# sherna90/dropout_hamiltonian_montecarlo

Hardware: AMD Instinct MI355X
Metric: leapfrog-steps/sec × param-dim, MNIST softmax SGHMC, 1/2/4/8 chains↔GPUs (higher is better)
Workload: dtype f64

## Files before the change

### dropout_hamiltonian_montecarlo_amd/_native.py

```python
import atexit
import ctypes
import os
import threading

import torch

_HERE = os.path.dirname(os.path.abspath(__file__))
LIB_PATH = os.path.join(_HERE, "lib", os.environ.get("HMCX_LIB", "libhmcx.so"))

HMCX_F32, HMCX_F64 = 0, 1
NOISE_BUFFER, NOISE_PHILOX = 0, 1

c_int, c_double, c_void_p = ctypes.c_int, ctypes.c_double, ctypes.c_void_p
c_i64p = ctypes.POINTER(ctypes.c_int64)
c_i32p = ctypes.POINTER(ctypes.c_int32)
c_dblp = ctypes.POINTER(ctypes.c_double)
c_u8p = ctypes.POINTER(ctypes.c_uint8)


class SamplerArgs(ctypes.Structure):
    _fields_ = [("dtype", c_int), ("B", c_int), ("D", c_int), ("K", c_int), ("C", c_int),
                ("n_steps", c_int), ("alpha", c_double), ("log_prior", c_double),
                ("X", c_void_p), ("Y", c_void_p), ("row0", c_void_p), ("eps", c_void_p),
                ("n_iter", c_void_p), ("u_accept", c_void_p), ("want_ll", c_void_p),
# ... 92 lines not shown
    _fields_ = [("dim", c_int), ("C", c_int), ("n_steps", c_int), ("mu", c_void_p), ("prec", c_void_p),
                ("nlp_const", c_double), ("mult", c_dblp), ("site", c_i32p), ("u_accept", c_dblp),
                ("noise_mode", c_int), ("noise", c_void_p), ("noise_off", c_i64p),
                ("seed", ctypes.c_uint64), ("chain0", ctypes.c_uint32), ("step_base", ctypes.c_uint32),
                ("x", c_void_p), ("out_A", c_void_p), ("out_accepted", c_void_p), ("out_logp", c_void_p),
                ("out_E", c_void_p), ("out_trace", c_void_p)]


MODEL_SOFTMAX, MODEL_LOGISTIC = 0, 1
MLP_MASK_SLOT0 = 0x80000000
MLP_MASKS_NONE, MLP_MASKS_FIXED, MLP_MASKS_PHILOX = 0, 1, 2


EXPORTS = ("hmcx_version", "hmcx_create", "hmcx_destroy", "hmcx_last_error", "hmcx_set_stream",
           "hmcx_synchronize", "hmcx_set_graph_mode", "hmcx_set_sghmc_path", "hmcx_set_timing", "hmcx_get_timing",
           "hmcx_philox_uniforms", "hmcx_philox_normals", "hmcx_philox_normals_f64",
           "hmcx_softmax_grad", "hmcx_softmax_loglik", "hmcx_softmax_predict", "hmcx_sghmc_run",
           "hmcx_sgld_run", "hmcx_hmc_mvn_run", "hmcx_mlp_masks", "hmcx_mlp_grad", "hmcx_mlp_loss",
           "hmcx_mlp_sghmc_run", "hmcx_mlp_hmc_leapfrog", "hmcx_mlp_predictive", "hmcx_logistic_grad", "hmcx_logistic_loglik", "hmcx_logistic_predict",
           "hmcx_sumsq", "hmcx_sgd_run", "hmcx_hmc_run", "hmcx_hmc_chains_run", "hmcx_mh_run", "hmcx_mh_mvn_run", "hmcx_axpy", "hmcx_mvn_eval",
           "hmcx_clear_abort", "hmcx_get_recoveries", "hmcx_note_recovery", "hmcx_get_mlp_forward_counts", "hmcx_set_sgld_fuse", "hmcx_philox_schedule", "hmcx_host_wait", "hmcx_set_mlp_fuse",
           "hmcx_comm_unique_id", "hmcx_comm_init", "hmcx_comm_destroy", "hmcx_allgather_chain_stats",
           "hmcx_allreduce_f64", "hmcx_chain_diagnostics", "hmcx_p2_plan_query", "hmcx_p2_ahead_query",
           "hmcx_set_sghmc_ahead", "hmcx_sghmc_ahead_note", "hmcx_p2_ahead_rule", "hmcx_sghmc_batch_plan_query")

_lib = None
_lock = threading.Lock()


class HmcxError(RuntimeError):
    pass


def load_library():
    global _lib
    with _lock:
        if _lib is not None:
            return _lib
        if not os.path.exists(LIB_PATH):
            raise HmcxError("libhmcx.so not built (%s): run `python -c 'import __graft_entry__ as g; g.build()'`"
                            % LIB_PATH)
        lib = ctypes.CDLL(LIB_PATH)
        lib.hmcx_version.restype = c_int
        lib.hmcx_create.argtypes = [c_int, ctypes.POINTER(c_void_p)]
        lib.hmcx_destroy.argtypes = [c_void_p]
        lib.hmcx_last_error.argtypes = [c_void_p]
        lib.hmcx_last_error.restype = ctypes.c_char_p
# ... 57 lines not shown
        lib.hmcx_logistic_grad.argtypes = [c_void_p, c_int, c_void_p, c_void_p, c_int, c_int, c_int,
                                           c_void_p, c_void_p, c_double, c_void_p, c_void_p]
        lib.hmcx_logistic_loglik.argtypes = [c_void_p, c_int, c_void_p, c_void_p, c_int, c_int, c_int,
                                             c_void_p, c_void_p, c_void_p]
        lib.hmcx_logistic_predict.argtypes = [c_void_p, c_int, c_void_p, c_int, c_int, c_int, c_void_p, c_void_p,
                                              c_void_p]
        lib.hmcx_sumsq.argtypes = [c_void_p, c_int, c_void_p, ctypes.c_int64, c_void_p]
        lib.hmcx_sgd_run.argtypes = [c_void_p, ctypes.POINTER(SgdArgs)]
        lib.hmcx_hmc_run.argtypes = [c_void_p, ctypes.POINTER(HmcArgs)]
        if hasattr(lib, "hmcx_hmc_chains_run"):
            lib.hmcx_hmc_chains_run.argtypes = [c_void_p, ctypes.POINTER(HmcChainsArgs)]
        if hasattr(lib, "hmcx_mh_run"):
            lib.hmcx_mh_run.argtypes = [c_void_p, ctypes.POINTER(MhArgs)]
            lib.hmcx_mh_mvn_run.argtypes = [c_void_p, ctypes.POINTER(MhMvnArgs)]
        if hasattr(lib, "hmcx_p2_plan_query"):
            lib.hmcx_p2_plan_query.argtypes = [c_int, c_int, c_int, c_int, c_int, ctypes.c_longlong, c_int, c_int,
                                               ctypes.POINTER(ctypes.c_longlong)]
        if hasattr(lib, "hmcx_set_sghmc_ahead"):
            lib.hmcx_set_sghmc_ahead.argtypes = [c_void_p, c_int]
            lib.hmcx_sghmc_ahead_note.argtypes = [c_void_p, c_i32p, c_int]
            lib.hmcx_p2_ahead_rule.argtypes = [c_int, c_int, c_int]
            lib.hmcx_p2_ahead_query.argtypes = [c_int, c_int, c_int, c_int, c_int, ctypes.c_longlong, c_int, c_int,
                                                ctypes.POINTER(ctypes.c_longlong)]
        if hasattr(lib, "hmcx_sghmc_batch_plan_query"):
            lib.hmcx_sghmc_batch_plan_query.argtypes = [c_int] * 11 + [ctypes.POINTER(ctypes.c_longlong)]
        lib.hmcx_axpy.argtypes = [c_void_p, c_int, c_int, ctypes.c_int64, c_double, c_void_p, c_void_p]
        lib.hmcx_mvn_eval.argtypes = [c_void_p, c_int, c_int, c_void_p, c_void_p, c_double, c_void_p, c_void_p,
                                      c_void_p]
        _lib = lib
        return lib


class Context:

    def __init__(self, device):
        lib = load_library()
        if not torch.cuda.is_available():
            raise HmcxError("no HIP device visible: the HIP engine has no CPU fallback")
        self.lib = lib
        self.device = torch.device("cuda", device if isinstance(device, int) else (device.index or 0))
        h = c_void_p()
        with torch.cuda.device(self.device):
            rc = lib.hmcx_create(self.device.index, ctypes.byref(h))
        if rc != 0:
            raise HmcxError("hmcx_create failed (%d)" % rc)
        self.h = h
# ... 11 lines not shown

    def check(self, rc, what):
        if rc != 0:
            msg = self.lib.hmcx_last_error(self.h)
            raise HmcxError("%s failed (%d): %s" % (what, rc, msg.decode() if msg else ""))

    path = 0

    def set_sghmc_path(self, path):
        self.check(self.lib.hmcx_set_sghmc_path(self.h, int(path)), "hmcx_set_sghmc_path")
        self.path = int(path)

    def set_sghmc_ahead(self, mode):
        self.check(self.lib.hmcx_set_sghmc_ahead(self.h, int(mode)), "hmcx_set_sghmc_ahead")

    def sghmc_ahead_note(self, accepted):
        if not hasattr(self.lib, "hmcx_sghmc_ahead_note"):
            return
        if hasattr(accepted, "ctypes") and accepted.dtype.str == "<i4" and accepted.flags.c_contiguous:
            self.lib.hmcx_sghmc_ahead_note(self.h, accepted.ctypes.data_as(c_i32p), int(accepted.size))
            return
        flags = [1 if v else 0 for v in accepted]
        self.lib.hmcx_sghmc_ahead_note(self.h, (ctypes.c_int32 * len(flags))(*flags), len(flags))

    def clear_abort(self):
        self.check(self.lib.hmcx_clear_abort(self.h), "hmcx_clear_abort")

    RECOVERY_KINDS = ("persistent_sghmc", "mlp_fused", "sgld_wide_fused")

    def recoveries(self):
        if not hasattr(self.lib, "hmcx_get_recoveries"):
            return None
        out = (ctypes.c_int64 * len(self.RECOVERY_KINDS))()
        self.check(self.lib.hmcx_get_recoveries(self.h, out), "hmcx_get_recoveries")
        return dict(zip(self.RECOVERY_KINDS, (int(v) for v in out)))

    def note_recovery(self, kind):
        self.check(self.lib.hmcx_note_recovery(self.h, self.RECOVERY_KINDS.index(kind)), "hmcx_note_recovery")

    MLP_FORWARD_KINDS = ("fwdr", "batched", "single")

    def mlp_forward_counts(self):
        out = (ctypes.c_int64 * len(self.MLP_FORWARD_KINDS))()
        self.check(self.lib.hmcx_get_mlp_forward_counts(self.h, out), "hmcx_get_mlp_forward_counts")
        return dict(zip(self.MLP_FORWARD_KINDS, (int(v) for v in out)))

# ... 155 lines not shown
```

### dropout_hamiltonian_montecarlo_amd/csrc/hmcx_ctx.hip

```cpp
#include "hmcx_common.h"
#include "hmcx_internal.h"
#include <new>
#include <cstdio>
#include <cstring>
#include <cmath>

namespace hmcx {

int set_error(hmcx_ctx* ctx, int code, const std::string& msg) {
  if (ctx) ctx->err = msg;
  return code;
}

bool Workspace::retry() {
  if (off <= ctx->ws_cap) return false;
  if (ctx->ws) {
    if (hipDeviceSynchronize() != hipSuccess) { failed = true; return false; }
    (void)hipFree(ctx->ws);
    ctx->ws = nullptr;
    ctx->ws_cap = 0;
  }
  const size_t want = off + off / 4 + (1 << 20);
  if (hipMalloc((void**)&ctx->ws, want) != hipSuccess) {
    ctx->ws = nullptr;
// ... 528 lines not shown
  return HMCX_OK;
}

int hmcx_destroy(hmcx_ctx* ctx) {
  HMCX_GUARD_CTX(ctx);
  (void)hipSetDevice(ctx->device);
  (void)hipStreamSynchronize(ctx->stream);
  if (ctx->ws) (void)hipFree(ctx->ws);
  for (int i = 0; i < 2; ++i) {
    if (ctx->stage_buf[i]) (void)hipHostFree(ctx->stage_buf[i]);
    if (ctx->stage_evv[i]) (void)hipEventDestroy(ctx->stage_evv[i]);
  }
  if (ctx->ev_in) (void)hipEventDestroy(ctx->ev_in);
  for (auto& pr : ctx->t_pend) { (void)hipEventDestroy(pr.first); (void)hipEventDestroy(pr.second); }
  if (ctx->t_open) (void)hipEventDestroy(ctx->t_open);
  for (auto& pr : ctx->abort_pend) (void)hipEventDestroy(pr.first);
  for (auto e : ctx->ev_pool) (void)hipEventDestroy(e);
  for (auto& m : ctx->host_marks) (void)hipEventDestroy(m.second);
  for (auto e : ctx->host_mark_pool) (void)hipEventDestroy(e);
  if (ctx->abort_host) (void)hipHostFree(ctx->abort_host);
  if (ctx->abort_dev) (void)hipFree(ctx->abort_dev);
  if (ctx->mlp_abort_dev) (void)hipFree(ctx->mlp_abort_dev);
  if (ctx->wide_abort_dev) (void)hipFree(ctx->wide_abort_dev);
  if (ctx->zeros_dev) (void)hipFree(ctx->zeros_dev);
  if (ctx->gx_arena) (void)hipFree(ctx->gx_arena);
  if (ctx->pred_ws) (void)hipFree(ctx->pred_ws);
  for (auto& g : ctx->graveyard) {
    (void)hipGraphExecDestroy(g.first);
    (void)hipEventDestroy(g.second);
  }
  if (ctx->own_stream) (void)hipStreamDestroy(ctx->own_stream);
  delete ctx;
  return HMCX_OK;
}

const char* hmcx_last_error(const hmcx_ctx* ctx) { return ctx ? ctx->err.c_str() : "null context"; }

int hmcx_set_stream(hmcx_ctx* ctx, void* stream) {
  HMCX_GUARD_CTX(ctx);
  ctx->stream = (hipStream_t)stream;
  return HMCX_OK;
}

int hmcx_synchronize(hmcx_ctx* ctx) {
  HMCX_GUARD_CTX(ctx);
  HMCX_HIP(ctx, hipStreamSynchronize(ctx->stream));
// ... 545 lines not shown
```

### dropout_hamiltonian_montecarlo_amd/csrc/hmcx_internal.h

```cpp
#pragma once
#include <hip/hip_runtime.h>
#include <stdint.h>
#include <string>
#include <vector>
#include <algorithm>
#include "hmcx.h"

struct hmcx_ctx {
  int device = 0;
  hipStream_t own_stream = nullptr;
  hipStream_t stream = nullptr;
  std::string err;
  int graph_mode = 0;
  int sghmc_path = 0;
  int sghmc_ahead = 2;
  int ahead_on = 1;
  uint64_t ahead_flags = 0;
  int ahead_seen = 0;
  int num_cus = 256;
  size_t lds_max = 160 * 1024;
  char* ws = nullptr;
  size_t ws_cap = 0;
  char* stage_buf[2] = {nullptr, nullptr};
  size_t stage_capv[2] = {0, 0};
  hipEvent_t stage_evv[2] = {nullptr, nullptr};
  bool stage_pend[2] = {false, false};
  int stage_cur = 0;
  size_t stage_off = 0;
  char* gx_arena = nullptr;
  size_t gx_bytes = 0;
  unsigned gx_epoch = 0;
  std::vector<int64_t> rs_poff, rs_nzo;
  std::vector<double> sched_L, sched_u;
  std::vector<int32_t> sched_n;
  std::vector<std::pair<std::pair<const void*, int>, int>> occ_cache;
  hipEvent_t ev_in = nullptr, ev_out = nullptr;
  std::vector<std::pair<hipGraphExec_t, hipEvent_t>> graveyard;
  int timing = 0;
  hipEvent_t t_open = nullptr;
  std::vector<std::pair<hipEvent_t, hipEvent_t>> t_pend;
  double t_ms = 0.0;
// ... 179 lines not shown
```

### dropout_hamiltonian_montecarlo_amd/csrc/hmcx_p2x.h

```cpp
#pragma once
#include "hmcx_common.h"

namespace hmcx {

constexpr int QTH = 256;
constexpr int QNW = QTH / 64;
constexpr int QNPM = 16;
#ifndef HMCX_P2_SLEEP
#define HMCX_P2_SLEEP 1
#endif
constexpr unsigned long long QTIMEOUT = 400000000ull;

typedef unsigned int gran_t __attribute__((ext_vector_type(4)));
__host__ __device__ inline int p2_pad(int n, int pad) { return pad ? (n + 7) & ~7 : n; }

__device__ inline uint64_t opaque_s64(uint64_t x) {
  uint32_t lo = (uint32_t)x, hi = (uint32_t)(x >> 32);
  asm volatile("" : "+s"(lo), "+s"(hi));
  return ((uint64_t)hi << 32) | lo;
}
__device__ inline int opaque(int x) {
  asm volatile("" : "+v"(x));
  return x;
}
// ... 235 lines not shown
}
__device__ inline int p2_wait_decision(unsigned long long* w, unsigned ep, int* abort_flag) {
  unsigned long long t0 = __builtin_amdgcn_s_memrealtime();
  for (int spins = 0;; ++spins) {
    const unsigned long long cur = __hip_atomic_load(w, __ATOMIC_RELAXED, __HIP_MEMORY_SCOPE_AGENT);
    if ((cur >> 2) == (unsigned long long)ep) return (int)(cur & 3ull);
    if ((spins & 63) == 63 &&
        (__builtin_amdgcn_s_memrealtime() - t0 > QTIMEOUT ||
         __hip_atomic_load(abort_flag, __ATOMIC_RELAXED, __HIP_MEMORY_SCOPE_AGENT))) {
      const int d = p2_decide(w, ep, P2_ABORT);
      if (d == P2_ABORT) p2_timeout(abort_flag, -1, ep);
      return d;
    }
    if (HMCX_P2_SLEEP) __builtin_amdgcn_s_sleep(1);
  }
}

__device__ inline bool all_ok(bool ok, int* sh_fail) {
  if (!ok) *sh_fail = 1;
  __syncthreads();
  return *sh_fail == 0;
}

__device__ inline double wsum(double v, double* sh) {
#pragma unroll
  for (int m = 32; m >= 1; m >>= 1) v += __shfl_xor(v, m, 64);
  if ((threadIdx.x & 63) == 0) sh[threadIdx.x >> 6] = v;
  __syncthreads();
  double r = sh[0];
#pragma unroll
  for (int w = 1; w < QNW; ++w) r += sh[w];
  __syncthreads();
  return r;
}

template <int CTRL> __device__ inline double dpp64(double v) {
  const unsigned long long x = __builtin_bit_cast(unsigned long long, v);
  const int lo = __builtin_amdgcn_mov_dpp((int)(unsigned)x, CTRL, 0xF, 0xF, false);
  const int hi = __builtin_amdgcn_mov_dpp((int)(unsigned)(x >> 32), CTRL, 0xF, 0xF, false);
  return __builtin_bit_cast(double, (unsigned long long)(unsigned)lo | ((unsigned long long)(unsigned)hi << 32));
}
template <int CTRL> __device__ inline float dpp64(float v) {
  return __builtin_bit_cast(float, __builtin_amdgcn_mov_dpp(__builtin_bit_cast(int, v), CTRL, 0xF, 0xF, false));
}
constexpr int DPP_XOR1 = 0xB1, DPP_XOR2 = 0x4E, DPP_HMIRROR = 0x141, DPP_MIRROR = 0x140;
template <typename T> __device__ inline T g16_max2(T v) {
// ... 18 lines not shown
```

### dropout_hamiltonian_montecarlo_amd/csrc/hmcx_persist2.hip

```cpp
#include "hmcx_common.h"
#include "hmcx_internal.h"
#include "hmcx_persist.h"
#include "hmcx_p2x.h"
#include <cstdio>
#include <cstdlib>
#include <vector>

namespace hmcx {


struct Q2Args {
  int B, D, K, P, n_steps;
  int Gr, Gf, Br, Bf, BfP, BFP, Ro, Fo;
  double alpha, neg_inv_n, log_prior;
  const void* X; const void* Y;
  const double* eps; const double* u; const int64_t* row0; const int32_t* n_iter;
  int noise_mode; const double* noise; const int64_t* noff;
  uint64_t seed; uint32_t chain0, step_base;
  void* W; void* b;
  char* arena;
  int oXA, oXD, oXB, oXW, oXS;
  int oXC;
  int oXAh, oXQ, oXP;
  int help;
// ... 1 lines not shown
  int pad;
  unsigned ep0;
  int zoff;
  int spread;
  int xmap;
  int fl2;
  int al2;
  int prefetch;
  int acc1;
  int bar;
  int* abort_flag;
  int force_abort;
  double* out_A; int32_t* out_acc; double* out_ll; double* out_E;
  void* out_trace;
  void* out_mom;
  unsigned long long* prof;
  unsigned long long* trace;
  int* verdict;
  int ninl;
  struct { double eps, u; int64_t row0; int32_t n_iter, pad_; } inl[32];
  int ahead;
  int laneoff;
  int oXV;
};
constexpr int P2_NINL = 32;
__device__ inline int sched_k(int s) { return s < P2_NINL ? s : P2_NINL - 1; }
template <typename V>
__device__ inline V sched_at(bool inl, int s, V kv, const V* g) {
  const V gv = g[inl ? 0 : s];
  return inl ? kv : gv;
}

struct P2Verdict {
  int* out;
  bool done;
  __device__ ~P2Verdict() {
    if (out && !done) out[0] = 1;
  }
};
constexpr int P2TR_IT = 16;
#ifndef HMCX_P2_HELP_DEFAULT
#define HMCX_P2_HELP_DEFAULT 2
#endif

struct P2Prof {
  unsigned long long* out;
// ... 395 lines not shown
      }
    }
    verdict.done = true;
    return;
  }

  const int s_first = lanei, s_inc = ah ? 2 : 1;
  bool redo = false;
  bool pf_done = false;
  int tb = 0;
  const int perV = p2_pad(Fo * KC + KC, pad);
  const auto gatherQ = [&](int k) -> bool {
    const int ni = Fo * KC + KC;
    const int base0 = a.oXQ + ((k & 1) * Gf + f) * Gr * perV;
    const bool ok = gather_ws(rs, base0, perV, Gr, ni, [](int i) { return i; },
                              [&](int p, int i) { return i < Fo * KC ? p * Fo + i / KC < nfeat : p == 0; },
                              a.ep0 + (unsigned)k, a.abort_flag, [&](int q, double v) {
      const int p = q / ni, i = q - p * ni;
      if (i < Fo * KC) Wf[(p * Fo + i / KC) * 16 + i % KC] = (T)v;
      else bsh[i - Fo * KC] = (T)v;
    });
    return all_ok(ok, ish);
  };
  const auto waitV = [&](int k) -> int {
    if (threadIdx.x == 0) {
      const int g = (a.oXV + ((k & 1) * G + pbid) * 8) * 16;
      const unsigned tg = a.ep0 + (unsigned)k;
      unsigned long long t0 = __builtin_amdgcn_s_memrealtime();
      int res = -1;
      for (int spins = 0;; ++spins) {
        const gran_t v = __builtin_amdgcn_raw_buffer_load_b128(rs, g, 0, 16 );
        if (pass_complete(gran_miss(v, tg))) { res = decode(v) != 0.0 ? 1 : 0; break; }
        if ((spins & 63) == 63 && p2_spin_over(t0, a.abort_flag, a.oXV, tg)) break;
        __builtin_amdgcn_s_sleep(4);
      }
      ish[2] = res;
    }
    __syncthreads();
    const int res = ish[2];
    __syncthreads();
    return res;
  };

  for (int s = s_first; s < a.n_steps;) {
    const int tid = opaque((int)threadIdx.x), lane = tid & 63, wave = tid >> 6, lr = lane & 15;
    const double epsd = sched_at(inl, s, a.inl[sched_k(s)].eps, a.eps);
    const T eps = (T)epsd, ome = (T)(1.0 - epsd), nsc = (T)(2.0 * epsd);
    const int n = sched_at(inl, s, a.inl[sched_k(s)].n_iter, a.n_iter);
    const int64_t rw = sched_at(inl, s, a.inl[sched_k(s)].row0, a.row0);
    const T* Xg = reinterpret_cast<const T*>(a.X) + (size_t)rw * D;
    const T* Yg = reinterpret_cast<const T*>(a.Y) + (size_t)rw * K;
    prof.stamp(0);
    if (s == a.force_abort && bid == G - 1) {
      if (tid == 0) __hip_atomic_store(a.abort_flag, 1, __ATOMIC_RELAXED, __HIP_MEMORY_SCOPE_AGENT);
      return;
    }

    if ((s == s_first || !prefetch) && !redo) load_step_rows<T>(Xc, Yc, Xg, Yg, Br, BfP, BFP, nrow, nfeat, row0, feat0, D, K, Ro, nro, ro0);
    for (int e = tid; e < BfP * 16; e += QTH) Wf0[e] = Wf[e];
    if (hp) {
      if (tid >= QTH - 16) b0sh[tid - (QTH - 16)] = bsh[tid - (QTH - 16)];
      if (s == 0) xp_issue(0, 0);
      for (int c = 0; c * 2 * QTH < nXPi; ++c) {
        if (c > 0) xp_issue(s, c);
        if (!all_ok(xp_finish(c, ep), ish)) return;
      }
      pw = own ? pWs[wl] : T(0);
      if (n > 0)
        for (int j = tid; j < nfeat * KC; j += QTH) {
          const int l = (j / KC) * 16 + (j - (j / KC) * KC);
          Wf[l] = Wf[l] + eps * pWs[l];
        }
    } else {
      pw = own ? noise1<T>(a, s, 0u, (uint32_t)e_own) : T(0);
// ... 45 lines not shown
        const double t = kv ? (double)(Yc[ii * 16 + k] * (z - lse)) : 0.0;
        const double rsum = g16_sum2(t);
        if (k == 0) rowll[ii] = rsum;
      }
      __syncthreads();
      if (tid == 0) {
        double v = 0.0;
        for (int ii = 0; ii < nro; ++ii) v += rowll[ii];
        dsh[4] = v;
      }
      __syncthreads();
      ll0 = dsh[4];
    }

    double kin1 = 0.0;
    T zb_prev = T(0);
    for (int it = 0; it < n; ++it) {
      const int tid = opaque((int)threadIdx.x), lane = tid & 63, wave = tid >> 6, lr = lane & 15;
      const bool last = it == n - 1;
      if (it == 0 && own) wv = wv + eps * pw;

      prof.stamp(1);
      const int parA = (int)(uA & 1);
      roundA(parA);
      tstamp(s, it, 0);
      if (bar && it > 0 && tid < K) {
        const T gr = -((T)hdr[tid] - alpha * bpsh[tid]);
        pbsh[tid] = (ome * pbsh[tid] + eps * gr) + nsc * zb_prev;
        bsh[tid] = bpsh[tid];
      }
      if (tid < 16) bpsh[tid] = bsh[tid] + eps * pbsh[tid];
      prof.stamp(2);
      T zb = T(0);
      if (zoff) {
        const int zi = tid - NZ0;
        if (zi >= 0 && zi < nfo * KC + K) {
          bool v = true;
          uint32_t e;
          if (zi < nfo * KC) {
            const int od_ = zi / KC, ok_ = zi - (zi / KC) * KC;
            v = ok_ < K;
            e = (uint32_t)((feat0 + fo0 + od_) * K + ok_);
          } else {
            e = (uint32_t)(D * K + zi - nfo * KC);
          }
          zbuf[zi] = v ? noise1<T>(a, s, (uint32_t)(it + 1), e) : T(0);
        }
      } else {
// ... 28 lines not shown
            Csr[ii * 16 + k] = dd;
            if (last) {
              const T lse = log(sm) + m;
              const double t = kv ? (double)(y * (z - lse)) : 0.0;
              const double rsum = g16_sum2(t);
              if (k == 0) rowll[ii] = rsum;
            }
          }
        }
        __syncthreads();
      }
      prof.stamp(5);
      double hv = 0.0;
      {
        ++ep;
        const int reg = oXD + (((int)(uD & 1) * Gr + r) * Gf + f) * NXA;
        for (int t = tid; t < NXA0; t += QTH) {
          double v;
          if (t < KC) {
            T c = T(0);
            for (int ii = 0; ii < nro; ++ii) c += Csr[ii * 16 + t];
            v = (double)c;
          } else if (t == KC) {
            v = 0.0;
            if (last) for (int ii = 0; ii < nro; ++ii) v += rowll[ii];
          } else {
            const int m = t - HA;
            v = (double)Dme[(m / KC) * 16 + (m % KC)];
          }
          put_t(al2, rs, reg + t, v, ep);
        }
        tstamp(s, it, 2);
        const int base0 = oXD + ((int)(uD & 1) * Gr + r) * Gf * NXA;
        ++uD;
        bool ok;
        if (spread & 2) {
          ok = gather_st(rs, base0, NXA, Gf, NXA0, [](int i) { return i; }, ep, a.abort_flag, [&](int q, double v) {
            const int p = q / NXA0, t = q - p * NXA0;
            if (t < HA) stg[q] = v;
            else Ds[(p * Ro + (t - HA) / KC) * 16 + (t - HA) % KC] = (T)v;
          });
          if (!all_ok(ok, ish)) return;
          if (tid < HA) {
            double hvs[QNPM];
#pragma unroll
            for (int p = 0; p < QNPM; ++p) hvs[p] = stg[min(p, Gf - 1) * NXA0 + tid];
            hv = hvs[0];
#pragma unroll
// ... 42 lines not shown
            T v = Zp[i * 16 + k];
            for (int q = 1; q < WPB; ++q) v += Zp[(q * BfP + i) * 16 + k];
            put_t(fl2, rs, reg + HA + e, bpart(i, k, (double)v), ep);
          }
        }
        const int base0 = oXB + ((int)(uB & 1) * Gf + f) * Gr * NXB;
        ++uB;
        tstamp(s, it, 4);
        prof.stamp(7);
        if (bar) {
          const int ni = HA + nfeat * KC;
          bool ok = true;
          double kl = 0.0;
          for (int i0 = tid; i0 < ni; i0 += 2 * QTH) {
            int off[2] = {i0, i0 + QTH};
            const unsigned vm = 1u | (off[1] < ni ? 2u : 0u);
            double sm[2];
            ok = polln<2>(rs, base0, NXB, Gr, off, vm, ep, sm, a.abort_flag, []() {});
            if (!ok) break;
#pragma unroll
            for (int j = 0; j < 2; ++j) {
              const int i = off[j];
              if (i >= ni) continue;
              if (i < HA) { hdr[i] = sm[j]; continue; }
              const int m = i - HA, d = m / KC, k = m - (m / KC) * KC;
              if (k >= K) continue;
              const int l = d * 16 + k;
              const T w = Wf[l];
              const T gz = -((T)sm[j] - alpha * w);
              const T p = ome * pWs[l] + eps * gz;
              pWs[l] = p;
              if (!last) Wf[l] = w + eps * p;
              else if (d >= fo0 && d < fo0 + nfo) kl += (double)p * (double)p;
            }
          }
          if (!all_ok(ok, ish)) return;
          tstamp(s, it, 5);
          prof.stamp(8);
          if (last) {
            if (tid < K) {
              const T gr = -((T)hdr[tid] - alpha * bpsh[tid]);
              pbsh[tid] = (ome * pbsh[tid] + eps * gr) + nsc * zb;
              bsh[tid] = bpsh[tid];
            }
            ll_last = hdr[KC];
            kin1 = kl;
            break;
          }
          zb_prev = zb;
          continue;
        }
        const int ng = nfo * KC;
        double sum = 0.0;
        const bool isg = tid < ng, ish_ = tid >= ng && tid < ng + HA;
        const int offB = isg ? HA + fo0 * KC + tid : tid - ng;
        if (spread & 4) {
          const int ni = ng + HA;
          const bool ok = gather(rs, base0, NXB, Gr, ni, [&](int i) { return i < ng ? HA + fo0 * KC + i : i - ng; },
                                 all_items, ep, a.abort_flag, stg);
          if (!all_ok(ok, ish)) return;
          if (tid < ni) {
            sum = stg[tid];
            for (int p = 1; p < Gr; ++p) sum += stg[p * ni + tid];
          }
          if (ish_) hdr[tid - ng] = sum;
          __syncthreads();
        } else {
          const bool ok = fl2 ? poll<true, double, 16>(rs, base0, NXB, Gr, -1, offB, isg || ish_, ep, nullptr, 0, &sum,
                                                        a.abort_flag)
                                : poll<true>(rs, base0, NXB, Gr, -1, offB, isg || ish_, ep, nullptr, 0, &sum, a.abort_flag);
          if (ish_) hdr[tid - ng] = sum;
          if (!all_ok(ok, ish)) return;
        }
        tstamp(s, it, 5);
        prof.stamp(8);
        if (own) {
          const T gr = -((T)sum - alpha * wv);
          const T p = (ome * pw + eps * gr) + nsc * zn;
          pw = p;
          if (!last) wv = wv + eps * p;
          else kin1 = (double)p * (double)p;
        }
        if (tid < K) {
          const T gr = -((T)hdr[tid] - alpha * bpsh[tid]);
          pbsh[tid] = (ome * pbsh[tid] + eps * gr) + nsc * zb;
          bsh[tid] = bpsh[tid];
        }
        if (last) ll_last = hdr[KC];
      }
      if (last) break;
      prof.stamp(9);
      {
        ++ep;
        const int per = p2_pad(Fo * KC, pad);
        const int reg = oXW + (((int)(uW & 1) * Gf + f) * Gr + r) * per;
        if (tid < nfo * KC) put_t(fl2, rs, reg + tid, own ? (double)wv : 0.0, ep);
        tstamp(s, it, 6);
        if (own) Wf[wl] = wv;
// ... 3 lines not shown
          const int ni = Fo * KC;
          const auto want = [&](int p, int i) { return p != r && p < min(Gr, (nfeat - i / KC + Fo - 1) / Fo); };
          const bool ok = gather(rs, base0, per, Gr, ni, [](int i) { return i; }, want, ep, a.abort_flag, stg);
          if (!all_ok(ok, ish)) return;
          for (int q = tid; q < Gr * ni; q += QTH) {
            const int p = q / ni, i = q - p * ni;
            if (want(p, i)) Wf[(p * Fo + i / KC) * 16 + i % KC] = (T)stg[q];
          }
          __syncthreads();
          tstamp(s, it, 7);
          continue;
        }
        const int dloc = tid / KC, kk = tid - (tid / KC) * KC;
        const int npd = tid < Fo * KC ? min(Gr, (nfeat - dloc + Fo - 1) / Fo) : 0;
        const bool ok = fl2 ? poll<false, T, 16>(rs, base0, per, npd, r, tid, tid < Fo * KC, ep, nullptr, 0, nullptr,
                                                  a.abort_flag, Wf + dloc * 16 + kk, Fo * 16)
                              : poll<false>(rs, base0, per, npd, r, tid, tid < Fo * KC, ep, nullptr, 0, nullptr,
                                            a.abort_flag, Wf + dloc * 16 + kk, Fo * 16);
        if (!all_ok(ok, ish)) return;
        tstamp(s, it, 7);
      }
    }

    if (bar && n > 0 && own) wv = Wf[wl];
    prof.stamp(10);
    const double kin1w = wsum(kin1, dsh);
    double kb1 = 0.0;
    for (int k = 0; k < K; ++k) kb1 += (double)pbsh[k] * (double)pbsh[k];
    ++ep;
    {
      const int reg = oXS + ((int)(uS & 1) * G + bid) * NXS;
      if (tid == 0) put(rs, reg + 0, kin0, ep);
      if (tid == 1) put(rs, reg + 1, kin1w, ep);
      if (tid == 2 && !hp) put(rs, reg + 2, ll0, ep);
    }
    if (hp && s + 1 < a.n_steps) xp_issue(s + 1, 0);
    if (prefetch && s + s_inc < a.n_steps && !pf_done) {
      const int sn = s + s_inc;
      const int64_t rn = sched_at(inl, sn, a.inl[sched_k(sn)].row0, a.row0);
      const T* Xn = reinterpret_cast<const T*>(a.X) + (size_t)rn * D;
      const T* Yn = reinterpret_cast<const T*>(a.Y) + (size_t)rn * K;
      load_step_rows<T>(ah ? (tb ? Xs : Xs2) : Xs, ah ? (tb ? Yo : Yo2) : Yo, Xn, Yn, Br, BfP, BFP, nrow, nfeat, row0, feat0,
                        D, K, Ro, nro, ro0);
      pf_done = ah;
    }
    const int sbase = oXS + (int)(uS & 1) * G * NXS;
// ... 9 lines not shown
#pragma unroll
      for (int j = 0; j < 3; ++j)
        ok = ok && poll<true>(rs, sbase + j, NXS, 1, -1, tid * NXS, tid < G, ep, nullptr, 0, &v3[j], a.abort_flag);
      if (!all_ok(ok, ish)) return;
    }
    const double S0 = wsum(v3[0], dsh), S1 = wsum(v3[1], dsh), L0 = wsum(v3[2], dsh);
    const double K0 = (0.0 + 0.5 * S0) + 0.5 * kb0;
    const double Ecur = a.neg_inv_n * (L0 + a.log_prior) + K0;
    double A, Enew, llq;
    int acc;
    if (n <= 0) {
      A = 1.0; Enew = Ecur; llq = L0;
      acc = sched_at(inl, s, a.inl[sched_k(s)].u, a.u) < A;
    } else {
      const double K1 = (0.0 + 0.5 * S1) + 0.5 * kb1;
      Enew = a.neg_inv_n * (ll_last + a.log_prior) + K1;
      const double x = exp(Ecur - Enew);
      A = (x < 1.0) ? x : 1.0;
      acc = sched_at(inl, s, a.inl[sched_k(s)].u, a.u) < A;
      llq = acc ? ll_last : L0;
    }
    if (ah && s > 0 && !redo) {
      prof.stamp(12);
      const int vprev = waitV(s - 1);
      if (vprev < 0) return;
      if (vprev) {
        prof.stamp(13);
        if (!gatherQ(s - 1)) return;
        wv = own ? Wf[wl] : T(0);
        redo = true;
        continue;
      }
    }
    if (!acc || n <= 0) {
      for (int e = tid; e < BfP * 16; e += QTH) Wf[e] = Wf0[e];
      wv = w0;
      if (tid < 16) bsh[tid] = b0sh[tid];
    }
    if (a.out_mom && s == a.n_steps - 1) {
      T* mo = reinterpret_cast<T*>(a.out_mom);
      const bool keep_new = acc && n > 0;
      if (own) mo[e_own] = keep_new ? (bar ? pWs[wl] : pw) : pw0;
      if (bid == 0 && tid < K) mo[D * K + tid] = keep_new ? pbsh[tid] : pb0sh[tid];
    }
    if (a.out_trace) {
      T* tr = reinterpret_cast<T*>(a.out_trace) + (size_t)s * (D * K + K);
      if (own) tr[e_own] = wv;
      if (bid == 0 && tid < K) tr[D * K + tid] = bsh[tid];
    }
    if (bid == 0 && tid == 0) {
// ... 9 lines not shown
      else if (r == 0 && tid < Fo * KC + KC) put_t(fl2, rs, reg + tid, (double)bsh[tid - Fo * KC], ep);
    }
    if (ah) {
      const bool changed = acc && n > 0;
      const unsigned tg = a.ep0 + (unsigned)s;
      if (changed && (s + 1 < a.n_steps || lanei)) {
        const int reg = a.oXQ + (((s & 1) * Gf + f) * Gr + r) * perV;
        if (tid < Fo * KC) put_t(fl2, rs, reg + tid, own ? (double)wv : 0.0, tg);
        else if (r == 0 && tid < Fo * KC + KC) put_t(fl2, rs, reg + tid, (double)bsh[tid - Fo * KC], tg);
      }
      if (tid == 0) put(rs, a.oXV + ((s & 1) * G + pbid) * 8, changed ? 1.0 : 0.0, tg);
      if (pf_done) {
        tb ^= 1;
        Xc = tb ? Xs2 : Xs;
        Yc = tb ? Yo2 : Yo;
        pf_done = false;
      }
      redo = false;
    }
    s += s_inc;
  }
  prof.stamp(0);
  prof.flush();
  if (ah) {
    if (lanei) {
      verdict.done = true;
      return;
    }
    if (a.n_steps >= 2 && !(a.n_steps & 1)) {
      const int vlast = waitV(a.n_steps - 1);
      if (vlast < 0) return;
      if (vlast) {
        if (!gatherQ(a.n_steps - 1)) return;
        wv = own ? Wf[wl] : T(0);
      }
    }
  }
  ++ep;
  if (tid == 0) put(rs, a.oXC + bid, 1.0, ep);
  {
    unsigned long long* dword = reinterpret_cast<unsigned long long*>(a.arena + (size_t)(a.oXC + G) * 16);
    if (bid == 0) {
      const bool ok = gather_st(rs, a.oXC, 1, G, 1, [](int) { return 0; }, ep, a.abort_flag, [](int, double) {});
      const bool all = all_ok(ok, ish);
      if (tid == 0) ish[1] = p2_decide(dword, ep, all ? P2_COMMIT : P2_ABORT);
    } else if (tid == 0) {
      ish[1] = p2_wait_decision(dword, ep, a.abort_flag);
    }
    __syncthreads();
    if (ish[1] != P2_COMMIT) return;
  }
  verdict.done = true;
  if (own) reinterpret_cast<T*>(a.W)[e_own] = wv;
// ... 176 lines not shown
  int64_t* d_noff = reinterpret_cast<int64_t*>(dp[4]);

  a.B = s->B; a.D = s->D; a.K = K; a.P = s->D * K + K; a.n_steps = s->n_steps;
  a.Gr = pl.Gr; a.Gf = pl.Gf; a.Br = pl.Br; a.Bf = pl.Bf; a.BfP = pl.BfP; a.BFP = pl.BFP; a.Ro = pl.Ro; a.Fo = pl.Fo;
  a.alpha = s->alpha; a.neg_inv_n = -1.0 / (double)s->B; a.log_prior = s->log_prior;
  a.X = s->X; a.Y = s->Y;
  a.eps = d_eps; a.u = d_u; a.row0 = d_row0; a.n_iter = d_n;
  if (a.ninl > 0) {
    a.eps = a.u = reinterpret_cast<double*>(ctx->zeros_dev);
    a.row0 = reinterpret_cast<int64_t*>(ctx->zeros_dev);
    a.n_iter = reinterpret_cast<int32_t*>(ctx->zeros_dev);
  }
  a.noise_mode = s->noise_mode; a.noise = s->noise; a.noff = d_noff;
  a.seed = s->seed; a.chain0 = s->chain0; a.step_base = s->step_base;
  a.W = s->W; a.b = s->b;
  a.arena = arena;
  a.oXA = (int)lay.oXA; a.oXD = (int)lay.oXD; a.oXB = (int)lay.oXB; a.oXW = (int)lay.oXW;
  a.oXS = (int)lay.oXS; a.oXC = (int)lay.oXC; a.oXAh = (int)lay.oXAh; a.oXQ = (int)lay.oXQ;
  a.oXP = (int)lay.oXP;
  a.help = help;
  a.ahead = ahead;
  a.laneoff = (int)(lay.oL1 - lay.oXA);
  a.oXV = (int)lay.oXV;
  a.arena_bytes = (int)(ngran * 16);
  a.ep0 = ep0;
  a.pad = pad;
  static const bool dbg = getenv("HMCX_P2_DEBUG") && getenv("HMCX_P2_DEBUG")[0] == '1';
  if (dbg)
    fprintf(stderr, "[hmcx p2] B=%d D=%d K=%d plan %dx%d Br=%d Bf=%d BfP=%d Ro=%d Fo=%d; granule bases XA %d XD %d XB %d "
            "XW %d XS %d XC %d; help %d XAh %d XQ %d XP %d; ahead %d lane-1 offset %d XV %d; epochs %u..%u\n", s->B, s->D, K,
            pl.Gr, pl.Gf, pl.Br, pl.Bf, pl.BfP, pl.Ro, pl.Fo, a.oXA, a.oXD, a.oXB, a.oXW, a.oXS, a.oXC, a.help, a.oXAh, a.oXQ,
            a.oXP, a.ahead, a.laneoff, a.oXV, ep0, ep0 + rounds - 1);
  {
    const int HA = KC + 1;
    const bool fits = pl.Gf * pl.Ro * KC <= QSTAGE && pl.Gf * (HA + pl.Ro * KC) <= QSTAGE &&
                      pl.Gr * (pl.Fo * KC + HA) <= QSTAGE && pl.Gr * pl.Fo * KC <= QSTAGE;
    static const int spread_env = getenv("HMCX_P2_SPREAD") ? atoi(getenv("HMCX_P2_SPREAD")) : 2;
    a.spread = fits ? spread_env : 0;
    a.zoff = !(getenv("HMCX_P2_ZOFF") && getenv("HMCX_P2_ZOFF")[0] == '0');
    static const int bar_env = getenv("HMCX_P2_BAR") ? atoi(getenv("HMCX_P2_BAR")) : 1;
    a.bar = bar_env == 1 ? 1 : 0;
    const int xmap_env = getenv("HMCX_P2_XMAP") ? atoi(getenv("HMCX_P2_XMAP")) : (a.bar ? 0 : 1);
    a.xmap = (xmap_env == 1 && (pl.Gr * pl.Gf) % 8 == 0) ? 1 : 0;
    static const int fl2_env = getenv("HMCX_P2_FL2") ? atoi(getenv("HMCX_P2_FL2")) : 1;
    a.fl2 = (fl2_env == 1 && !a.xmap && pl.Gf % 8 == 0 && xmap_env != 2) ? 1 : 0;
    a.al2 = (fl2_env == 1 && a.xmap && ((pl.Gr * pl.Gf) / 8) % pl.Gf == 0) ? 1 : 0;
// ... 62 lines not shown
    if (!dprof && !dtrace) return HMCX_OK;
  } else if (s->out_host) {
    char* h = reinterpret_cast<char*>(s->out_host);
    const bool packed = s->out_abort == reinterpret_cast<int32_t*>(reinterpret_cast<char*>(s->out_A) + 36 * n);
    HMCX_HIP(ctx, hipMemcpyAsync(h, s->out_A, 36 * n + (packed ? sizeof(int) : 0), hipMemcpyDeviceToHost,
                                 ctx->stream));
    if (!packed)
      HMCX_HIP(ctx, hipMemcpyAsync(h + 36 * n, s->out_abort ? (const void*)s->out_abort : ctx->abort_dev,
                                   sizeof(int), hipMemcpyDeviceToHost, ctx->stream));
    if (!dprof && !dtrace) return HMCX_OK;
  }
  if (s->out_abort) {
    if (!dprof && !dtrace) return HMCX_OK;
  } else if (!dprof && !dtrace) {
    return abort_defer(ctx, a.abort_flag, ctx->stream);
  }
  int flag = 0;
  HMCX_HIP(ctx, hipMemcpyAsync(&flag, a.abort_flag, sizeof(int), hipMemcpyDeviceToHost, ctx->stream));
  HMCX_HIP(ctx, hipStreamSynchronize(ctx->stream));
  if (dprof) {
    unsigned long long hh[32];
    HMCX_HIP(ctx, hipMemcpy(hh, dprof, sizeof(hh), hipMemcpyDeviceToHost));
    (void)hipFree(dprof);
    static const char* names[14] = {"step-start", "A-gemm+publish", "noise", "A-RS wait", "softmax", "A-AG",
                                    "B-gemm+publish", "B-RS wait", "update", "B-AG", "accept", "it=-1",
                                    "verdict wait+apply", "state gather"};
    for (int ln = 0; ln < (ahead ? 2 : 1); ++ln) {
      const unsigned long long* h = hh + 16 * ln;
      unsigned long long tot = 0;
      for (int i = 0; i < 14; ++i) tot += h[i];
      fprintf(stderr, "[hmcx p2 prof] G=%dx%d Br=%d Bf=%d Ro=%d Fo=%d lane %d total %llu ticks:", pl.Gr, pl.Gf, pl.Br,
              pl.Bf, pl.Ro, pl.Fo, ln, tot);
      for (int i = 0; i < 14; ++i) fprintf(stderr, " %s %.1f%%", names[i], tot ? 100.0 * h[i] / tot : 0.0);
      fprintf(stderr, "\n");
    }
  }
  if (dtrace) {
    std::vector<unsigned long long> h(ntr);
    HMCX_HIP(ctx, hipMemcpy(h.data(), dtrace, ntr * sizeof(unsigned long long), hipMemcpyDeviceToHost));
    (void)hipFree(dtrace);
    static const char* rn[4] = {"A-RS", "A-AG", "B-RS", "B-AG"};
    for (int rd = 0; rd < 4; ++rd) {
      double lat = 0, skew = 0, lmax = 0;
      long cnt = 0;
      for (int it = 1; it < P2TR_IT; ++it)
        for (int b = 0; b < G; ++b) {
          const int r = b / pl.Gf, f = b % pl.Gf;
          const unsigned long long pub = h[((size_t)b * P2TR_IT + it) * 8 + 2 * rd];
          const unsigned long long done = h[((size_t)b * P2TR_IT + it) * 8 + 2 * rd + 1];
          if (!pub || !done) continue;
          unsigned long long mx = 0;
          const bool rowteam = rd < 2;
          const int nm = rowteam ? pl.Gf : pl.Gr;
          bool okm = true;
          for (int m = 0; m < nm; ++m) {
            const int pb = rowteam ? r * pl.Gf + m : m * pl.Gf + f;
// ... 33 lines not shown
                         (long long)(help ? 2 : 1) * p.Gr * p.Gf,
                         l.oXA, l.nXA, l.oXD, l.nXD, l.oXB, l.nXB, l.oXW, l.nXW, l.oXS, l.nXS, l.oXC, l.nXC, l.oXAh, l.nXAh,
                         l.oXQ, l.nXQ, l.oXP, l.nXP, l.ngran};
  for (int i = 0; i < 30; ++i) out[1 + i] = v[i];
  return 0;
}

extern "C" int hmcx_p2_ahead_query(int B, int D, int K, int tsize, int num_cus, long long lds_max, int pad, int want,
                                   long long* out) {
  using namespace hmcx;
  const PersistPlan2 p = plan_p2(B, D, K, (size_t)tsize, num_cus, (size_t)lds_max);
  for (int i = 0; i < 26; ++i) out[i] = 0;
  if (!p.ok) return 0;
  size_t lds = p.lds;
  const int ahead = p2_ahead_mode(p, K, (size_t)tsize, num_cus, (size_t)lds_max, want, &lds);
  const P2Layout l = p2_layout(p, K, pad, 0, ahead);
  const long long v[] = {ahead, (long long)(ahead ? 2 : 1) * p.Gr * p.Gf, (long long)lds, (long long)p.lds,
                         l.oXA, l.nXA, l.oXD, l.nXD, l.oXB, l.nXB, l.oXW, l.nXW, l.oXS, l.nXS, l.oXC, l.nXC,
                         l.oXQ, l.nXQ, l.oL1, l.nL1, l.oXV, l.nXV, l.ngran, p.Br, p.BFP, p.Ro};
  for (int i = 0; i < 26; ++i) out[i] = v[i];
  return 0;
}

extern "C" int hmcx_p2_ahead_rule(int on, int seen, int accepted) {
  if (seen < hmcx::P2_AHEAD_MIN) return on ? 1 : 0;
  const double rate = (double)accepted / (double)seen;
  if (on && rate > hmcx::P2_AHEAD_OFF_ABOVE) return 0;
  if (!on && rate < hmcx::P2_AHEAD_ON_BELOW) return 1;
  return on ? 1 : 0;
}

namespace hmcx {

template int sghmc_p2_t<float>(hmcx_ctx*, const hmcx_sampler_args*, const PersistPlan2&);
template int sghmc_p2_t<double>(hmcx_ctx*, const hmcx_sampler_args*, const PersistPlan2&);

}
```

### include/hmcx.h

```cpp
#ifndef HMCX_H
#define HMCX_H
#include <stdint.h>

#ifdef __cplusplus
extern "C" {
#endif

typedef struct hmcx_ctx hmcx_ctx;

enum hmcx_dtype { HMCX_F32 = 0, HMCX_F64 = 1 };
enum hmcx_noise { HMCX_NOISE_BUFFER = 0, HMCX_NOISE_PHILOX = 1 };
enum hmcx_status {
  HMCX_OK = 0,
  HMCX_EINVAL = -1,
  HMCX_EHIP = -2,
  HMCX_ENOMEM = -3,
  HMCX_EUNSUPPORTED = -4
};

int hmcx_version(void);
int hmcx_create(int device, hmcx_ctx** out);
int hmcx_destroy(hmcx_ctx* ctx);
const char* hmcx_last_error(const hmcx_ctx* ctx);
int hmcx_set_stream(hmcx_ctx* ctx, void* hip_stream);
int hmcx_synchronize(hmcx_ctx* ctx);
int hmcx_set_graph_mode(hmcx_ctx* ctx, int enabled);
int hmcx_set_sghmc_path(hmcx_ctx* ctx, int path);
int hmcx_set_sghmc_ahead(hmcx_ctx* ctx, int mode);
int hmcx_sghmc_ahead_note(hmcx_ctx* ctx, const int32_t* accepted , int n);
int hmcx_p2_ahead_rule(int on, int seen, int accepted);
int hmcx_set_timing(hmcx_ctx* ctx, int enabled);
int hmcx_get_timing(hmcx_ctx* ctx, double* kernel_ms, long long* launches);

void hmcx_philox_uniforms(uint64_t seed, uint32_t chain, uint32_t step, uint32_t slot,
                          uint32_t n, double* out );
void hmcx_philox_normals(uint64_t seed, uint32_t chain, uint32_t step, uint32_t slot,
                         uint32_t e0, uint32_t n, double* out );
void hmcx_philox_normals_f64(uint64_t seed, uint32_t chain, uint32_t step, uint32_t slot,
                             uint32_t e0, uint32_t n, double* out );

int hmcx_softmax_grad(hmcx_ctx* ctx, int dtype, const void* X, const void* Y, int B, int D, int K,
                      int C, const void* W, const void* b, double alpha, void* gW, void* gb);

int hmcx_softmax_loglik(hmcx_ctx* ctx, int dtype, const void* X, const void* Y, int B, int D, int K,
                        int C, const void* W, const void* b, double* ll);

int hmcx_softmax_predict(hmcx_ctx* ctx, int dtype, const void* X, int B, int D, int K, int C,
                         const void* W, const void* b, void* prob);

int hmcx_logistic_grad(hmcx_ctx* ctx, int dtype, const void* X, const void* y, int B, int D, int C,
                       const void* W, const void* b, double alpha, void* gW, void* gb);
int hmcx_logistic_loglik(hmcx_ctx* ctx, int dtype, const void* X, const void* y, int B, int D, int C,
                         const void* W, const void* b, double* ll);
// ... 322 lines not shown
```

Baseline: 1.396 billion.

## Abort speculative run-ahead SGHMC step early once previous step's verdict requires redo

In the persistent two-lane SGHMC kernel with run-ahead, the speculative step now polls the previous step's accept verdict during the leapfrog loop. The verdict is broadcast through the reduce-scatter header slot, so all blocks can stop the remaining leapfrog iterations as soon as a redo is known, instead of finishing the whole wasted trajectory before redoing. It adjusts the epoch counter for the skipped iterations and adds device-side counters plus a host query for redo/stop/skip statistics. The cost is an extra buffer load and shared-memory flag checks per iteration, plus more complex epoch bookkeeping that could desynchronise blocks if it is wrong.

```diff
diff --git a/dropout_hamiltonian_montecarlo_amd/_native.py b/dropout_hamiltonian_montecarlo_amd/_native.py
--- a/dropout_hamiltonian_montecarlo_amd/_native.py
+++ b/dropout_hamiltonian_montecarlo_amd/_native.py
@@ -138,7 +138,8 @@
            "hmcx_clear_abort", "hmcx_get_recoveries", "hmcx_note_recovery", "hmcx_get_mlp_forward_counts", "hmcx_set_sgld_fuse", "hmcx_philox_schedule", "hmcx_host_wait", "hmcx_set_mlp_fuse",
            "hmcx_comm_unique_id", "hmcx_comm_init", "hmcx_comm_destroy", "hmcx_allgather_chain_stats",
            "hmcx_allreduce_f64", "hmcx_chain_diagnostics", "hmcx_p2_plan_query", "hmcx_p2_ahead_query",
-           "hmcx_set_sghmc_ahead", "hmcx_sghmc_ahead_note", "hmcx_p2_ahead_rule", "hmcx_sghmc_batch_plan_query")
+           "hmcx_set_sghmc_ahead", "hmcx_sghmc_ahead_note", "hmcx_p2_ahead_rule", "hmcx_sghmc_batch_plan_query",
+           "hmcx_sghmc_ahead_stats")
 
 _lib = None
 _lock = threading.Lock()
@@ -242,6 +243,8 @@
             lib.hmcx_p2_ahead_rule.argtypes = [c_int, c_int, c_int]
             lib.hmcx_p2_ahead_query.argtypes = [c_int, c_int, c_int, c_int, c_int, ctypes.c_longlong, c_int, c_int,
                                                 ctypes.POINTER(ctypes.c_longlong)]
+        if hasattr(lib, "hmcx_sghmc_ahead_stats"):
+            lib.hmcx_sghmc_ahead_stats.argtypes = [c_void_p, ctypes.POINTER(ctypes.c_longlong)]
         if hasattr(lib, "hmcx_sghmc_batch_plan_query"):
             lib.hmcx_sghmc_batch_plan_query.argtypes = [c_int] * 11 + [ctypes.POINTER(ctypes.c_longlong)]
         lib.hmcx_axpy.argtypes = [c_void_p, c_int, c_int, ctypes.c_int64, c_double, c_void_p, c_void_p]
@@ -299,6 +302,13 @@
             return
         flags = [1 if v else 0 for v in accepted]
         self.lib.hmcx_sghmc_ahead_note(self.h, (ctypes.c_int32 * len(flags))(*flags), len(flags))
+
+    def sghmc_ahead_stats(self):
+        if not hasattr(self.lib, "hmcx_sghmc_ahead_stats"):
+            return None
+        out = (ctypes.c_longlong * 3)()
+        self.check(self.lib.hmcx_sghmc_ahead_stats(self.h, out), "hmcx_sghmc_ahead_stats")
+        return {"redone": int(out[0]), "stopped": int(out[1]), "skipped": int(out[2])}
 
     def clear_abort(self):
         self.check(self.lib.hmcx_clear_abort(self.h), "hmcx_clear_abort")
diff --git a/dropout_hamiltonian_montecarlo_amd/csrc/hmcx_ctx.hip b/dropout_hamiltonian_montecarlo_amd/csrc/hmcx_ctx.hip
--- a/dropout_hamiltonian_montecarlo_amd/csrc/hmcx_ctx.hip
+++ b/dropout_hamiltonian_montecarlo_amd/csrc/hmcx_ctx.hip
@@ -574,6 +574,7 @@
   if (ctx->abort_dev) (void)hipFree(ctx->abort_dev);
   if (ctx->mlp_abort_dev) (void)hipFree(ctx->mlp_abort_dev);
   if (ctx->wide_abort_dev) (void)hipFree(ctx->wide_abort_dev);
+  if (ctx->ahead_stats_dev) (void)hipFree(ctx->ahead_stats_dev);
   if (ctx->zeros_dev) (void)hipFree(ctx->zeros_dev);
   if (ctx->gx_arena) (void)hipFree(ctx->gx_arena);
   if (ctx->pred_ws) (void)hipFree(ctx->pred_ws);
diff --git a/dropout_hamiltonian_montecarlo_amd/csrc/hmcx_internal.h b/dropout_hamiltonian_montecarlo_amd/csrc/hmcx_internal.h
--- a/dropout_hamiltonian_montecarlo_amd/csrc/hmcx_internal.h
+++ b/dropout_hamiltonian_montecarlo_amd/csrc/hmcx_internal.h
@@ -17,6 +17,8 @@
   int ahead_on = 1;
   uint64_t ahead_flags = 0;
   int ahead_seen = 0;
+  int* ahead_stats_dev = nullptr;
+  int ahead_stats_on = 0;
   int num_cus = 256;
   size_t lds_max = 160 * 1024;
   char* ws = nullptr;
diff --git a/dropout_hamiltonian_montecarlo_amd/csrc/hmcx_p2x.h b/dropout_hamiltonian_montecarlo_amd/csrc/hmcx_p2x.h
--- a/dropout_hamiltonian_montecarlo_amd/csrc/hmcx_p2x.h
+++ b/dropout_hamiltonian_montecarlo_amd/csrc/hmcx_p2x.h
@@ -281,6 +281,13 @@
   return *sh_fail == 0;
 }
 
+__device__ inline int all_okq(bool ok, int* sh) {
+  if (!ok) sh[0] = 1;
+  __syncthreads();
+  const int fail = sh[0], q = sh[1];
+  return fail ? -1 : q;
+}
+
 __device__ inline double wsum(double v, double* sh) {
 #pragma unroll
   for (int m = 32; m >= 1; m >>= 1) v += __shfl_xor(v, m, 64);
diff --git a/dropout_hamiltonian_montecarlo_amd/csrc/hmcx_persist2.hip b/dropout_hamiltonian_montecarlo_amd/csrc/hmcx_persist2.hip
--- a/dropout_hamiltonian_montecarlo_amd/csrc/hmcx_persist2.hip
+++ b/dropout_hamiltonian_montecarlo_amd/csrc/hmcx_persist2.hip
@@ -47,6 +47,7 @@
   int ahead;
   int laneoff;
   int oXV;
+  int* stats;
 };
 constexpr int P2_NINL = 32;
 __device__ inline int sched_k(int s) { return s < P2_NINL ? s : P2_NINL - 1; }
@@ -488,13 +489,13 @@
     });
     return all_ok(ok, ish);
   };
-  const auto waitV = [&](int k) -> int {
+  const auto waitV = [&](int k, int known) -> int {
     if (threadIdx.x == 0) {
       const int g = (a.oXV + ((k & 1) * G + pbid) * 8) * 16;
       const unsigned tg = a.ep0 + (unsigned)k;
       unsigned long long t0 = __builtin_amdgcn_s_memrealtime();
-      int res = -1;
-      for (int spins = 0;; ++spins) {
+      int res = known;
+      for (int spins = 0; known < 0; ++spins) {
         const gran_t v = __builtin_amdgcn_raw_buffer_load_b128(rs, g, 0, 16 );
         if (pass_complete(gran_miss(v, tg))) { res = decode(v) != 0.0 ? 1 : 0; break; }
         if ((spins & 63) == 63 && p2_spin_over(t0, a.abort_flag, a.oXV, tg)) break;
@@ -508,6 +509,8 @@
     return res;
   };
 
+  int c_redo = 0, c_stop = 0, c_skip = 0;
+  const bool cnt0 = ah && bid == 0 && threadIdx.x == 0;
   for (int s = s_first; s < a.n_steps;) {
     const int tid = opaque((int)threadIdx.x), lane = tid & 63, wave = tid >> 6, lr = lane & 15;
     const double epsd = sched_at(inl, s, a.inl[sched_k(s)].eps, a.eps);
@@ -516,6 +519,10 @@
     const int64_t rw = sched_at(inl, s, a.inl[sched_k(s)].row0, a.row0);
     const T* Xg = reinterpret_cast<const T*>(a.X) + (size_t)rw * D;
     const T* Yg = reinterpret_cast<const T*>(a.Y) + (size_t)rw * K;
+    const bool specrun = ah && s > 0 && !redo && n > 0;
+    int vst = -1;
+    int stopj = 0;
+    if (specrun && tid == 0) { ish[1] = 0; ish[3] = 0; }
     prof.stamp(0);
     if (s == a.force_abort && bid == G - 1) {
       if (tid == 0) __hip_atomic_store(a.abort_flag, 1, __ATOMIC_RELAXED, __HIP_MEMORY_SCOPE_AGENT);
@@ -607,8 +614,15 @@
 
       prof.stamp(1);
       const int parA = (int)(uA & 1);
+      const bool vlook = specrun && tid == 0 && vst < 0;
+      gran_t vq = {0u, 0u, 0u, 0u};
+      if (vlook) vq = __builtin_amdgcn_raw_buffer_load_b128(rs, (a.oXV + (((s - 1) & 1) * G + pbid) * 8) * 16, 0, 16 );
       roundA(parA);
       tstamp(s, it, 0);
+      if (vlook && pass_complete(gran_miss(vq, a.ep0 + (unsigned)(s - 1)))) {
+        vst = decode(vq) != 0.0 ? 1 : 0;
+        if (vst) ish[3] = 1;
+      }
       if (bar && it > 0 && tid < K) {
         const T gr = -((T)hdr[tid] - alpha * bpsh[tid]);
         pbsh[tid] = (ome * pbsh[tid] + eps * gr) + nsc * zb_prev;
@@ -683,8 +697,8 @@
             for (int ii = 0; ii < nro; ++ii) c += Csr[ii * 16 + t];
             v = (double)c;
           } else if (t == KC) {
-            v = 0.0;
-            if (last) for (int ii = 0; ii < nro; ++ii) v += rowll[ii];
+            v = (specrun && ish[3]) ? 1.0 : 0.0;
+            if (last) { v = 0.0; for (int ii = 0; ii < nro; ++ii) v += rowll[ii]; }
           } else {
             const int m = t - HA;
             v = (double)Dme[(m / KC) * 16 + (m % KC)];
@@ -773,7 +787,11 @@
             for (int j = 0; j < 2; ++j) {
               const int i = off[j];
               if (i >= ni) continue;
-              if (i < HA) { hdr[i] = sm[j]; continue; }
+              if (i < HA) {
+                hdr[i] = sm[j];
+                if (specrun && !last && i == KC && sm[j] != 0.0) ish[1] = 1;
+                continue;
+              }
               const int m = i - HA, d = m / KC, k = m - (m / KC) * KC;
               if (k >= K) continue;
               const int l = d * 16 + k;
@@ -785,9 +803,11 @@
               else if (d >= fo0 && d < fo0 + nfo) kl += (double)p * (double)p;
             }
           }
-          if (!all_ok(ok, ish)) return;
+          const int q = specrun ? all_okq(ok, ish) : all_ok(ok, ish) ? 0 : -1;
+          if (q < 0) return;
           tstamp(s, it, 5);
           prof.stamp(8);
+          if (q > 0 && !last) { stopj = it + 1; break; }
           if (last) {
             if (tid < K) {
               const T gr = -((T)hdr[tid] - alpha * bpsh[tid]);
@@ -825,6 +845,7 @@
         }
         tstamp(s, it, 5);
         prof.stamp(8);
+        if (specrun && !last && hdr[KC] != 0.0) { stopj = it + 1; break; }
         if (own) {
           const T gr = -((T)sum - alpha * wv);
           const T p = (ome * pw + eps * gr) + nsc * zn;
@@ -874,6 +895,15 @@
       }
     }
 
+    if (specrun && stopj) {
+      prof.stamp(14);
+      ep += (bar ? 3u : 4u) * (unsigned)(n - stopj) + 1u;
+      if (cnt0) { ++c_redo; ++c_stop; c_skip += n - stopj; }
+      if (!gatherQ(s - 1)) return;
+      wv = own ? Wf[wl] : T(0);
+      redo = true;
+      continue;
+    }
     if (bar && n > 0 && own) wv = Wf[wl];
     prof.stamp(10);
     const double kin1w = wsum(kin1, dsh);
@@ -929,10 +959,11 @@
     }
     if (ah && s > 0 && !redo) {
       prof.stamp(12);
-      const int vprev = waitV(s - 1);
+      const int vprev = waitV(s - 1, vst);
       if (vprev < 0) return;
       if (vprev) {
         prof.stamp(13);
+        if (cnt0) ++c_redo;
         if (!gatherQ(s - 1)) return;
         wv = own ? Wf[wl] : T(0);
         redo = true;
@@ -988,13 +1019,17 @@
   }
   prof.stamp(0);
   prof.flush();
+  if (cnt0 && a.stats) {
+    int* st = a.stats + 4 * lanei;
+    st[0] = c_redo; st[1] = c_stop; st[2] = c_skip;
+  }
   if (ah) {
     if (lanei) {
       verdict.done = true;
       return;
     }
     if (a.n_steps >= 2 && !(a.n_steps & 1)) {
-      const int vlast = waitV(a.n_steps - 1);
+      const int vlast = waitV(a.n_steps - 1, -1);
       if (vlast < 0) return;
       if (vlast) {
         if (!gatherQ(a.n_steps - 1)) return;
@@ -1217,6 +1252,12 @@
   a.ahead = ahead;
   a.laneoff = (int)(lay.oL1 - lay.oXA);
   a.oXV = (int)lay.oXV;
+  if (!ctx->ahead_stats_dev) {
+    HMCX_HIP(ctx, hipMalloc((void**)&ctx->ahead_stats_dev, 8 * sizeof(int)));
+    HMCX_HIP(ctx, hipMemsetAsync(ctx->ahead_stats_dev, 0, 8 * sizeof(int), ctx->stream));
+  }
+  a.stats = ctx->ahead_stats_dev;
+  ctx->ahead_stats_on = ahead;
   a.arena_bytes = (int)(ngran * 16);
   a.ep0 = ep0;
   a.pad = pad;
@@ -1325,16 +1366,16 @@
     unsigned long long hh[32];
     HMCX_HIP(ctx, hipMemcpy(hh, dprof, sizeof(hh), hipMemcpyDeviceToHost));
     (void)hipFree(dprof);
-    static const char* names[14] = {"step-start", "A-gemm+publish", "noise", "A-RS wait", "softmax", "A-AG",
+    static const char* names[15] = {"step-start", "A-gemm+publish", "noise", "A-RS wait", "softmax", "A-AG",
                                     "B-gemm+publish", "B-RS wait", "update", "B-AG", "accept", "it=-1",
-                                    "verdict wait+apply", "state gather"};
+                                    "verdict wait+apply", "state gather", "stopped run"};
     for (int ln = 0; ln < (ahead ? 2 : 1); ++ln) {
       const unsigned long long* h = hh + 16 * ln;
       unsigned long long tot = 0;
-      for (int i = 0; i < 14; ++i) tot += h[i];
+      for (int i = 0; i < 15; ++i) tot += h[i];
       fprintf(stderr, "[hmcx p2 prof] G=%dx%d Br=%d Bf=%d Ro=%d Fo=%d lane %d total %llu ticks:", pl.Gr, pl.Gf, pl.Br,
               pl.Bf, pl.Ro, pl.Fo, ln, tot);
-      for (int i = 0; i < 14; ++i) fprintf(stderr, " %s %.1f%%", names[i], tot ? 100.0 * h[i] / tot : 0.0);
+      for (int i = 0; i < 15; ++i) fprintf(stderr, " %s %.1f%% (%llu)", names[i], tot ? 100.0 * h[i] / tot : 0.0, h[i]);
       fprintf(stderr, "\n");
     }
   }
@@ -1414,6 +1455,18 @@
   return 0;
 }
 
+extern "C" int hmcx_sghmc_ahead_stats(hmcx_ctx* ctx, long long out[3]) {
+  if (!ctx) return HMCX_EINVAL;
+  if (!out) return hmcx::set_error(ctx, HMCX_EINVAL, "ahead_stats: null output");
+  out[0] = out[1] = out[2] = 0;
+  if (!ctx->ahead_stats_dev || !ctx->ahead_stats_on) return HMCX_OK;
+  int h[8];
+  HMCX_HIP(ctx, hipMemcpyAsync(h, ctx->ahead_stats_dev, sizeof(h), hipMemcpyDeviceToHost, ctx->stream));
+  HMCX_HIP(ctx, hipStreamSynchronize(ctx->stream));
+  for (int i = 0; i < 3; ++i) out[i] = (long long)h[i] + h[4 + i];
+  return HMCX_OK;
+}
+
 extern "C" int hmcx_p2_ahead_rule(int on, int seen, int accepted) {
   if (seen < hmcx::P2_AHEAD_MIN) return on ? 1 : 0;
   const double rate = (double)accepted / (double)seen;
diff --git a/include/hmcx.h b/include/hmcx.h
--- a/include/hmcx.h
+++ b/include/hmcx.h
@@ -29,6 +29,7 @@
 int hmcx_set_sghmc_ahead(hmcx_ctx* ctx, int mode);
 int hmcx_sghmc_ahead_note(hmcx_ctx* ctx, const int32_t* accepted , int n);
 int hmcx_p2_ahead_rule(int on, int seen, int accepted);
+int hmcx_sghmc_ahead_stats(hmcx_ctx* ctx, long long out[3]);
 int hmcx_set_timing(hmcx_ctx* ctx, int enabled);
 int hmcx_get_timing(hmcx_ctx* ctx, double* kernel_ms, long long* launches);
 
```

After: 1.485 billion, median of 6. +6.4%, better.
